# achilleasa/polaris

Hardware: AMD Instinct MI355X
Metric: Mrays/s (primary+indirect+occlusion rays traced / wall), Cornell box 512x512x128spp (higher is better)
Workload: dtype f32

## Files before the change

### polaris_amd/csrc/kernels.h

```cpp
#pragma once

#include <hip/hip_runtime.h>

#include <type_traits>

#include "builtin_probe.h"
#include "denoise.h"
#include "scene_layout.h"
#include "shading.h"
#include "temporal.h"
#include "variance.h"

namespace pol {

constexpr int WG = 256;
constexpr int kExitMarker = (int)0x80000000;

__device__ __forceinline__ float rcp_det(float x) {
	const float r = __builtin_amdgcn_rcpf(x);
	return __builtin_fmaf(__builtin_fmaf(-x, r, 1.0f), r, r);
}


__device__ __forceinline__ void rcp_dir(float dx, float dy, float dz, float &ix, float &iy, float &iz) {
// ... 1051 lines not shown
		uint32_t canon = 0;
		bool shade = tid < todo_rays;
		if (shade) canon = FIRST ? tid : canonical_index(pmask, (uint32_t)fbits(t4.w));
		if (!SORT && shade && A.prefilter) {
			const uint32_t fate = shade_fate(S, A, seed, [&]() { return pfx0 + canon; }, t4, h4.w);
			shade = fate == kFateLive;
			R.hit = fate == kFateRejected ? 1u : 0u;
		}
		if (shade) {
			shade_ray(S, A, s, seed, pfx0 + canon, d4, t4, h4, R, [&](float4 oo, float4 od, float4 oe) {
				const unsigned long long m = __ballot(true);
				const int first = __ffsll((long long)m) - 1;
				uint32_t at = 0;
				if ((int)lane == first) at = atomicAdd(&s_tot[1], (uint32_t)__popcll(m));
				const size_t d = base + (uint32_t)__builtin_amdgcn_readlane((int)at, first) + __popcll(m & below);
				st.occ_o[d] = oo; st.occ_d[d] = od; st.occ_e[d] = oe;
			});
		}
		const unsigned long long m_ind = __ballot(R.emit_ind);
		const unsigned long long mh = __ballot(R.hit != 0), mm = __ballot(R.miss != 0), me = __ballot(R.emit != 0);
		uint32_t at_ind = 0;
		if (lane == 0) {
			if (m_ind) at_ind = atomicAdd(&s_tot[0], (uint32_t)__popcll(m_ind));
			if (mh) atomicAdd(&s_tot[2], (uint32_t)__popcll(mh));
			if (mm) atomicAdd(&s_tot[3], (uint32_t)__popcll(mm));
			if (me) atomicAdd(&s_tot[4], (uint32_t)__popcll(me));
		}
		at_ind = __builtin_amdgcn_readfirstlane(at_ind);
		if (R.emit_ind) {
			atomicOr(&s_emit[canon >> 5], 1u << (canon & 31));
			const size_t d = base + at_ind + __popcll(m_ind & below);
			R.thr.w = ibits((int)canon);
			store_ray_o(st, d, R.ro); st.ray_d[d] = R.rd; st.thr[d] = R.thr;
		}
	}
	__threadfence_block();
	uint32_t arrived = 0;
	if (lane == 0) arrived = atomicAdd(&s_tot[5], 1u);
	if (__builtin_amdgcn_readfirstlane(arrived) == 3u) {
		__threadfence_block();
		if (lane == 0) {
			st.cnt_ray[blockIdx.x] = s_tot[0];
			st.cnt_occ[blockIdx.x] = s_tot[1];
			st.wg_stat[blockIdx.x] = s_tot[2] | (s_tot[3] << 10) | (s_tot[4] << 20);
		}
		if (lane < 8) A.emask_out[(size_t)blockIdx.x * 8 + lane] = s_emit[lane];
	}
}

constexpr int kSparseGroup = 8;
constexpr uint32_t kWaveQueue = 128;
static_assert(kWaveQueue >= 127 && (kWaveQueue & (kWaveQueue - 1)) == 0, "63 descriptors left by a shade pass + 64 of a screen pass; a ring indexed by masking");
static_assert(kSparseGroup <= 256 && WG <= 256, "a descriptor is chunk in group << 16 | slot << 8 | canonical index");
template <bool LDS>
__global__ __launch_bounds__(WG) __attribute__((amdgpu_waves_per_eu(4, 4)))
void k_shade_wave(Streams st, SceneDev Sg, ShadeArgs A, uint32_t num_chunks) {
	constexpr int G = kSparseGroup;
	__shared__ ShadeLds lds;
	__shared__ uint32_t wg_cursor;
	__shared__ uint32_t w_emit[4][G][8];
	__shared__ uint32_t w_cnt[4][G][3];
	__shared__ uint32_t w_queue[4][kWaveQueue];
	if (threadIdx.x == 0) wg_cursor = 0;
	for (uint32_t i = threadIdx.x; i < 4 * G * 8; i += WG) (&w_emit[0][0][0])[i] = 0;
	for (uint32_t i = threadIdx.x; i < 4 * G * 3; i += WG) (&w_cnt[0][0][0])[i] = 0;
	const SceneT<LDS> S = stage_scene<LDS>(Sg, lds);
	const uint32_t lane = threadIdx.x & 63, wave = threadIdx.x >> 6;
	const unsigned long long below = (1ull << lane) - 1ull;
	const uint32_t wgs_per_sample = A.Npad / WG;
	const uint32_t num_groups = (num_chunks + G - 1) / G;
	for (;;) {
		uint32_t c = 0;
		if (lane == 0) c = atomicAdd(&wg_cursor, 1u);
		const uint32_t group = blockIdx.x + __builtin_amdgcn_readfirstlane(c) * gridDim.x;
		if (group >= num_groups) break;
		const uint32_t chunk0 = group * G;
		const uint32_t my_cnt = (lane < (uint32_t)G && chunk0 + lane < num_chunks) ? st.cnt_ray[chunk0 + lane] : 0u;
		uint32_t incl = my_cnt;
#pragma unroll
		for (int d = 1; d < G; d <<= 1) {
			const uint32_t up = __shfl_up(incl, d);
			if ((int)lane >= d) incl += up;
		}
		const uint32_t excl = incl - my_cnt;
		const uint32_t total = (uint32_t)__builtin_amdgcn_readlane((int)incl, G - 1);
		uint32_t q_head = 0, q_tail = 0;
		auto shade_pass = [&]() {
			const uint32_t n = min(q_tail - q_head, 64u);
			const bool live = lane < n;
			__builtin_amdgcn_fence(__ATOMIC_RELEASE, "wavefront");
			__builtin_amdgcn_wave_barrier();
			__builtin_amdgcn_fence(__ATOMIC_ACQUIRE, "wavefront");
			const uint32_t desc = live ? w_queue[wave][(q_head + lane) & (kWaveQueue - 1)] : 0u;
			q_head += n;
			const uint32_t k = desc >> 16, idx = (desc >> 8) & 255u, canon = desc & 255u;
			const uint32_t chunk = chunk0 + k;
			const size_t base = (size_t)chunk * WG;
			ShadeOut R;
			R.emit_ind = false;
			R.hit = R.miss = R.emit = 0;
			if (live) {
				const uint32_t s = chunk / wgs_per_sample;
				const uint32_t seed = A.seeds[(size_t)(A.first_sample + s) * A.seed_stride + 1 + A.bounce];
				shade_ray(S, A, s, seed, st.pfx[chunk] + canon, st.ray_d[base + idx], st.thr[base + idx], load_hit(st, base + idx), R, [&](float4 oo, float4 od, float4 oe) {
					const size_t d = base + atomicAdd(&w_cnt[wave][k][1], 1u);
					st.occ_o[d] = oo; st.occ_d[d] = od; st.occ_e[d] = oe;
				});
			}
			if (R.emit_ind) {
				atomicOr(&w_emit[wave][k][canon >> 5], 1u << (canon & 31));
				const size_t d = base + atomicAdd(&w_cnt[wave][k][0], 1u);
				R.thr.w = ibits((int)canon);
				store_ray_o(st, d, R.ro); st.ray_d[d] = R.rd; st.thr[d] = R.thr;
			}
			if (live && (R.hit | R.miss | R.emit) != 0) atomicAdd(&w_cnt[wave][k][2], R.hit | (R.miss << 10) | (R.emit << 20));
		};
		for (uint32_t j = 0; j < total; j += 64) {
			const uint32_t r = j + lane;
			uint32_t k = 0, first = 0;
#pragma unroll
			for (int q = 1; q < G; q++) {
				const uint32_t e = (uint32_t)__builtin_amdgcn_readlane((int)excl, q);
				if (r >= e) { k = q; first = e; }
			}
			bool keep = false;
			uint32_t desc = 0;
			if (r < total) {
				const uint32_t chunk = chunk0 + k, idx = r - first;
				const size_t base = (size_t)chunk * WG;
				const float4 t4 = st.thr[base + idx];
				const uint4 m0 = reinterpret_cast<const uint4 *>(A.emask_in)[(size_t)chunk * 2], m1 = reinterpret_cast<const uint4 *>(A.emask_in)[(size_t)chunk * 2 + 1];
				const uint32_t pmask[8] = {m0.x, m0.y, m0.z, m0.w, m1.x, m1.y, m1.z, m1.w};
				const uint32_t canon = canonical_index(pmask, (uint32_t)fbits(t4.w));
				uint32_t fate = kFateLive;
				if (A.prefilter) {
					const uint32_t seed = A.seeds[(size_t)(A.first_sample + chunk / wgs_per_sample) * A.seed_stride + 1 + A.bounce];
					fate = shade_fate(S, A, seed, [&]() { return st.pfx[chunk] + canon; }, t4, load_hit_word(st, base + idx));
				}
				if (fate == kFateRejected) atomicAdd(&w_cnt[wave][k][2], 1u);
				keep = fate == kFateLive;
				desc = k << 16 | idx << 8 | canon;
			}
			const unsigned long long mk = __ballot(keep);
			if (keep) w_queue[wave][(q_tail + (uint32_t)__popcll(mk & below)) & (kWaveQueue - 1)] = desc;
			q_tail += (uint32_t)__popcll(mk);
			if (q_tail - q_head >= 64u) shade_pass();
		}
		if (q_tail != q_head) shade_pass();
		if (lane < (uint32_t)G && chunk0 + lane < num_chunks) {
			st.cnt_ray[chunk0 + lane] = w_cnt[wave][lane][0];
			st.cnt_occ[chunk0 + lane] = w_cnt[wave][lane][1];
			st.wg_stat[chunk0 + lane] = w_cnt[wave][lane][2];
			w_cnt[wave][lane][0] = 0; w_cnt[wave][lane][1] = 0; w_cnt[wave][lane][2] = 0;
		}
		for (uint32_t i = lane; i < (uint32_t)G * 8; i += 64) {
			if (chunk0 + i / 8 < num_chunks) A.emask_out[(size_t)chunk0 * 8 + i] = (&w_emit[wave][0][0])[i];
			(&w_emit[wave][0][0])[i] = 0;
		}
	}
}

enum ProbeKind { kProbeBxdf = 0, kProbeTexture = 1, kProbeEmissive = 2, kProbeMaterial = 3 };
constexpr uint32_t kProbeIn[4] = {13, 2, 11, 8}, kProbeOut[4] = {11, 7, 9, 18};

template <bool LDS>
__global__ __launch_bounds__(WG) void k_probe(SceneDev Sg, int kind, uint32_t index, uint32_t n, const float *in, float *out) {
	__shared__ ShadeLds lds;
	const SceneT<LDS> S = stage_scene<LDS>(Sg, lds);
	const uint32_t i = blockIdx.x * WG + threadIdx.x;
	if (i >= n) return;
	if (kind == kProbeBxdf) {
		const float *p = in + (size_t)i * 13;
		float *o = out + (size_t)i * 11;
		Surf sf;
		sf.p = splat(0.0f); sf.n = mk3(p[0], p[1], p[2]); sf.uv = {p[3], p[4]};
		const f3 wi = mk3(p[5], p[6], p[7]), wo = mk3(p[10], p[11], p[12]);
		MatT<LDS> m;
		m.nd = S.nodes + index;
		m.type = m.nd->type;
		m.int_ior = m.nd->int_ior; m.ext_ior = m.nd->ext_ior;
		material_params(sf, m, S);
		f3 dir = splat(0.0f);
		float pdf = 0.0f;
		const f3 v = bxdf_sample(sf, m, S, f2{p[8], p[9]}, wi, dir, pdf);
		float pdf2;
		f3 ev;
		bxdf_pdf_eval(sf, m, S, wi, wo, true, pdf2, ev);
		o[0] = v.x; o[1] = v.y; o[2] = v.z; o[3] = dir.x; o[4] = dir.y; o[5] = dir.z; o[6] = pdf;
		o[7] = pdf2; o[8] = ev.x; o[9] = ev.y; o[10] = ev.z;
	} else if (kind == kProbeTexture) {
		const float *p = in + (size_t)i * 2;
		float *o = out + (size_t)i * 7;
		const TexQuad q = tex_fetch(f2{p[0], p[1]}, (int)index, S);
		const f3 c = quad_sample3(q), b = quad_bump3(q);
		o[0] = c.x; o[1] = c.y; o[2] = c.z; o[3] = c.x; o[4] = b.x; o[5] = b.y; o[6] = b.z;
	} else if (kind == kProbeMaterial) {
		const float *p = in + (size_t)i * 8;
		float *o = out + (size_t)i * 18;
		Surf sf;
		sf.p = splat(0.0f); sf.n = mk3(p[0], p[1], p[2]); sf.uv = {p[3], p[4]};
		Rng rng = {(uint32_t)fbits(p[5]), (uint32_t)fbits(p[6])};
		uint32_t flags = (uint32_t)fbits(p[7]);
		f3 tint = splat(1.0f);
		const MatT<LDS> m = select_material(index, sf, flags, tint, rng, S);
		o[0] = ibits((int)m.type); o[1] = m.int_ior; o[2] = m.ext_ior;
		o[3] = sf.n.x; o[4] = sf.n.y; o[5] = sf.n.z; o[6] = tint.x; o[7] = tint.y; o[8] = tint.z;
		o[9] = ibits((int)flags); o[10] = ibits((int)rng.sx); o[11] = ibits((int)rng.sy);
		for (int k = 0; k < 3; k++) { o[12 + k] = m.nd->k[k]; o[15 + k] = m.nd->t[k]; }
// ... 486 lines not shown
```

### polaris_amd/csrc/polaris_hip.hip

```cpp
#include <hip/hip_runtime.h>

#include <algorithm>
#include <atomic>
#include <chrono>
#include <condition_variable>
#include <cmath>
#include <cstdarg>
#include <cstdio>
#include <cstdlib>
#include <cstring>
#include <map>
#include <memory>
#include <mutex>
#include <string>
#include <vector>

#include <unistd.h>

#include "camera_state.h"
#include "device_mem.h"
#include "frame_sync.h"
#include "kernel_table.h"
#include "merge_plan.h"
#include "polaris_hip.h"
// ... 233 lines not shown
	}
};

}

struct polaris_hip_tracer {
	int device = 0;
	char pci_bus_id[32] = {};
	hipStream_t stream = nullptr;
	std::mutex mu;
	std::string error;
	uint64_t error_seq = 0;

	FrameAccum fa;
	DevArray<uchar4> framebuffer;

	DeviceScene ds;
	int opt_node_mode = -1;
	int opt_tiny_one = 1;
	int opt_lds_tris = -1;

	CameraState camera;

	FrameSync fs;
	int opt_instance_update = 0, opt_vertex_update = 0;
	std::atomic<bool> opt_moments{false};

	struct Pipe {
		DevStream q;
		size_t slots = 0;
		Streams st{};
		float4 *nee[POLARIS_MAX_BOUNCES] = {};
		uint8_t *vis[POLARIS_MAX_BOUNCES] = {};
		uint32_t *cnt_occ_b[POLARIS_MAX_BOUNCES] = {};
		uint32_t nee_bounces = 0;
		DevPool bufs;
		DevEvent done;
		void release() {
			bufs.clear();
			st = Streams{};
			slots = 0;
			nee_bounces = 0;
			for (auto &x : nee) x = nullptr;
			for (auto &x : vis) x = nullptr;
			for (auto &x : cnt_occ_b) x = nullptr;
		}
	};
	static constexpr int kMaxPipes = pol::kMaxPipes;
	Pipe pipe[kMaxPipes];
	DevArray<uint32_t> d_seeds;
	DevArray<unsigned long long> d_stats;
	DevArray<float4> d_cam_o;
	int num_cus = 256;
	DevArray<uint32_t> d_retag;

	TraceOptions opt;
	bool packet_primary = true;
	int opt_time_kernels = 0;
	int opt_max_leaf_tris = -1;

	struct Pending { const char *name; DevEvent a, b; };
	std::vector<Pending> pending;
	std::vector<Pending> merge_pending;
	std::vector<DevEvent> event_pool;
	std::map<std::string, KernelTimer> timers;
	std::map<std::string, const char *> timer_symbol;
	int last_shade_timer[POLARIS_MAX_BOUNCES] = {};
	uint64_t last_shade_counts[3 * POLARIS_MAX_BOUNCES] = {};
	DevEvent ev_start, ev_stop, ev_fork;
};

struct polaris_hip_peer {
	polaris_hip_tracer *owner = nullptr;
	uint32_t depth = 0, W = 0, H = 0;
	IpcMapping mem[POLARIS_IPC_MAX_DEPTH];
	DevEvent ev[POLARIS_IPC_MAX_DEPTH];
	PolarisPeerInfo info{};
	void drop_events() { for (auto &e : ev) e.reset(); }
};


namespace {

int fail(polaris_hip_tracer *h, int code, const char *fmt, ...) {
	char buf[1024];
	va_list ap;
	va_start(ap, fmt);
	vsnprintf(buf, sizeof buf, fmt, ap);
	va_end(ap);
	if (h) { h->error = buf; h->error_seq = ++g_error_seq; }
	g_thread_error = buf;
	return code;
}

#define HIP_TRY(h, expr)                                                                              \
	do {                                                                                              \
		hipError_t e_ = (expr);                                                                       \
		if (e_ != hipSuccess) return fail(h, POLARIS_E_DEVICE, "%s failed: %s", #expr, hipGetErrorString(e_)); \
	} while (0)

template <typename T>
int dev_alloc(polaris_hip_tracer *h, DevPool &pool, T **out, size_t count) {
	DevArray<char> a;
	HIP_TRY(h, a.alloc(std::max<size_t>(count * sizeof(T), 16)));
	*out = (T *)a.get();
	pool.push_back(std::move(a));
// ... 194 lines not shown
	const bool tiny = h->ds.node_mode == kNodesLdsAll;
	for (int any = 0; any < 2; any++)
		h->ds.trace[any] = TraceLaunch{tiny ? &kTraceTiny[any][h->ds.tiny_one] : &kTrace[any][h->ds.max_stack <= 16 ? 0 : (h->ds.max_stack <= 24 ? 1 : 2)][h->ds.node_mode == kNodesLdsTop],
		                            tiny ? kTinyBlock : WG, 0, 6};
}

hipError_t launch_trace(polaris_hip_tracer *h, const char *timer, bool any_hit, hipStream_t q, Streams st, uint32_t grid, uint32_t chunks, float4 *acc, bool camera = false) {
	const TraceLaunch &T = h->ds.trace[any_hit];
	uint32_t o_mask = ~0u;
	if (camera && !any_hit) { st.ray_o = h->d_cam_o; o_mask = 0u; }
	return launch(h, timer, q, *T.v, grid, (uint32_t)T.block, T.lds_bytes, st, h->ds.bvh, chunks, acc, h->d_stats, o_mask);
}

int plan_tiny_lds(polaris_hip_tracer *h, size_t n_slots) {
	const uint32_t rows = (uint32_t)std::max(1, h->ds.max_stack - (h->ds.bvh.root_is_instance ? 1 : 0));
	constexpr uint32_t kRowBytes = kTinyBlock * (uint32_t)sizeof(int16_t), kTriBytes = 9 * sizeof(float) + sizeof(uint32_t);
	const uint32_t nodes = h->ds.bvh.num_pairs * (uint32_t)sizeof(PairNode);
	hipDeviceProp_t prop;
	size_t lds_per_cu = 160 * 1024;
	if (hipGetDeviceProperties(&prop, h->device) == hipSuccess && prop.maxSharedMemoryPerMultiProcessor > 0) lds_per_cu = prop.maxSharedMemoryPerMultiProcessor;
	const size_t half = lds_per_cu / 2;
	const size_t slack = 256;
	auto stack_off = [&](uint32_t tris) { return std::max<uint32_t>(kRowBytes, (nodes + tris * kTriBytes + 15u) & ~15u); };
	if (stack_off(0) + rows * kRowBytes + slack > half) return fail(h, POLARIS_E_DEVICE, "tiny-scene mode: stack and tree do not fit half a CU's LDS (%zu bytes)", half);
	uint32_t tris = (uint32_t)std::min<size_t>(n_slots, (half - slack - rows * kRowBytes - nodes - 16) / kTriBytes);
	if (tris < n_slots / 2) tris = 0;
	if (h->opt_lds_tris >= 0) tris = std::min<uint32_t>(tris, (uint32_t)h->opt_lds_tris);
	for (;;) {
		h->ds.bvh.tiny_stack_off = stack_off(tris);
		h->ds.bvh.lds_tris = tris;
		h->ds.trace[0].lds_bytes = h->ds.trace[1].lds_bytes = h->ds.bvh.tiny_stack_off + rows * kRowBytes;
		int worst = 8;
		for (const TraceLaunch &T : h->ds.trace) {
			HIP_TRY(h, hipFuncSetAttribute(T.v->address(), hipFuncAttributeMaxDynamicSharedMemorySize, (int)(half - slack)));
			int n = 0;
			if (hipOccupancyMaxActiveBlocksPerMultiprocessor(&n, T.v->address(), T.block, T.lds_bytes) != hipSuccess) { (void)hipGetLastError(); n = 2; }
			worst = std::min(worst, n);
		}
		if (worst >= 2 || tris == 0) break;
		tris = tris > 32 ? tris - 32 : 0;
	}
	if (getenv("POLARIS_DEBUG")) fprintf(stderr, "[polaris] tiny mode: %u stack rows at %u, %u pair records, %u of %zu triangle records in LDS (%u bytes per workgroup)\n", rows, h->ds.bvh.tiny_stack_off, h->ds.bvh.num_pairs, h->ds.bvh.lds_tris, n_slots, h->ds.trace[0].lds_bytes);
	return POLARIS_OK;
}

int trace_occupancy(polaris_hip_tracer *h, bool any_hit) {
	const TraceLaunch &T = h->ds.trace[any_hit];
	int n = 0;
	if (hipOccupancyMaxActiveBlocksPerMultiprocessor(&n, T.v->address(), T.block, T.lds_bytes) != hipSuccess || n < 1) n = h->ds.node_mode == kNodesLdsAll ? 1 : (h->ds.max_stack <= 24 ? 6 : 5);
	if (getenv("POLARIS_DEBUG")) fprintf(stderr, "[polaris] k_trace<%d> node mode %d: %d resident workgroups of %d threads per CU\n", (int)any_hit, h->ds.node_mode, n, T.block);
	return std::min(n, 8);
}

TraceScene plan_scene(const polaris_hip_tracer *h) {
	TraceScene s;
	s.tiny = h->ds.node_mode == kNodesLdsAll;
	for (int any = 0; any < 2; any++) s.resident_per_cu[any] = h->ds.trace[any].resident_per_cu;
	s.tables_fit_lds = h->ds.scene.num_nodes <= kLdsMatNodes && h->ds.scene.num_emissives <= kLdsLights && h->ds.scene.num_textures <= kLdsTextures;
	s.emit_classes = h->ds.scene.emit_classes;
	s.tri_bits = h->ds.scene.tri_bits;
	s.packet_primary = h->packet_primary;
	s.num_cus = h->num_cus;
	s.lens = h->camera.lens_on();
	s.shutter = h->camera.shutter_on();
	return s;
}

hipError_t launch_traversal(polaris_hip_tracer *h, const char *timer, Traversal how, RayKind kind, hipStream_t q, const Streams &st, uint32_t persistent_grid, uint32_t chunks, float4 *acc) {
	const bool any_hit = kind == RayKind::AnyHit;
	if (how == Traversal::Packet)
		return launch(h, timer, q, kPacket[any_hit ? kPacketAnyHit : (kind == RayKind::Camera ? kPacketCamera : kPacketClosest)], chunks, WG, 0, st, h->ds.bvh, acc, h->d_stats, make_float3(h->camera.open.eye[0], h->camera.open.eye[1], h->camera.open.eye[2]));
	if (how == Traversal::Persistent) return launch_trace(h, timer, any_hit, q, st, persistent_grid, chunks, acc, kind == RayKind::Camera);
	if (any_hit) return launch(h, timer, q, kOcclusion, chunks, WG, 0, st, h->ds.bvh, acc, h->d_stats);
	return launch(h, timer, q, kIntersect, chunks, WG, 0, st, h->ds.bvh);
}

hipError_t launch_generate(polaris_hip_tracer *h, const char *timer, hipStream_t q, const Streams &st, uint32_t stride, uint32_t first_sample, uint32_t wgs, uint32_t N,
                           uint32_t Npad, uint32_t block_y, int zero_lsum, int write_origin) {
	const CameraDev c = camera_args(h);
	const uint32_t *seeds = h->d_seeds;
	switch (const Generator g = h->camera.generator()) {
	case Generator::Pinhole: return launch(h, timer, q, kGenerate, wgs, WG, 0, st, c.cam, seeds, stride, first_sample, N, Npad, h->fa.W, block_y, zero_lsum, write_origin);
	case Generator::Lens: return launch(h, timer, q, kGenerateLens, wgs, WG, 0, st, c.cam, c.lens, seeds, stride, first_sample, N, Npad, h->fa.W, block_y, zero_lsum);
	default: return launch(h, timer, q, kGenerateShutter[g == Generator::ShutterLens], wgs, WG, 0, st, c.cam, c.cam1, c.lens, c.lens1, seeds, stride, first_sample, N, Npad, h->fa.W, block_y, zero_lsum);
	}
}

const char *const kShadeTimer[4] ={"shade_first", "shade_sort", "shade_plain", "shade_wave"};

hipError_t launch_batch(polaris_hip_tracer *h, int p, const PolarisBlockRequest *r, const TracePlan &plan, uint32_t s0, uint32_t K, uint32_t N, hipEvent_t resolve_after) {
	hipError_t first_err = hipSuccess;
	auto note = [&](hipError_t e) { if (first_err == hipSuccess && e != hipSuccess) first_err = e; };
	polaris_hip_tracer::Pipe &P = h->pipe[p];
	const bool exact = plan.exact;
	const uint32_t B = plan.bounces, stride = 1 + B, Npad = plan.Npad;
	const uint32_t wgs_per_sample = Npad / WG, wgs = K * wgs_per_sample;
	hipStream_t q = P.q;
	P.st.hit12 = plan.hit12 ? 1u : 0u;
	P.st.o12 = plan.o12 ? 1u : 0u;
	note(launch_generate(h, "generate", q, P.st, stride, s0, wgs, N, Npad, r->block_y, exact ? 0 : 1, plan.generate_writes_origins ? 1 : 0));
	ShadeArgs A{};
	A.seeds = h->d_seeds; A.seed_stride = stride; A.first_sample = s0;
	A.N = N; A.Npad = Npad; A.W = h->fa.W; A.blockY = r->block_y;
	A.min_rr = r->min_bounces_for_rr;
	A.exact = exact ? 1 : 0;
	A.prefilter = plan.prefilter ? 1 : 0;
	A.acc = exact ? h->fa.current() : P.st.lsum;
	const uint32_t persistent = plan.trace_grid(false, wgs), persistent_occl = plan.trace_grid(true, wgs);
	for (uint32_t b = 0; b < B; b++) {
		const BouncePlan &pl = plan.bounce[b];
		Streams S = P.st;
		if (!exact) { S.occ_e = P.nee[b]; S.vis = P.vis[b]; S.cnt_occ = P.cnt_occ_b[b]; }
		float4 *const occl_acc = exact ? A.acc : nullptr;
		const RayKind closest = b == 0 ? plan.primary : RayKind::Closest;
		note(launch_traversal(h, traversal_timer(pl.isect, closest), pl.isect, closest, q, S, persistent, wgs, nullptr));
// ... 238 lines not shown
	if (!out) return fail(nullptr, POLARIS_E_BAD_ARGUMENT, "device_identity: out is null");
	if (out->struct_size != sizeof(PolarisDeviceIdentity))
		return fail(nullptr, POLARIS_E_BAD_ARGUMENT, "device_identity: struct_size %u, this library's PolarisDeviceIdentity has %zu bytes", out->struct_size, sizeof(PolarisDeviceIdentity));
	const int n = polaris_hip_device_count();
	if (index < 0 || index >= n) return fail(nullptr, POLARIS_E_NO_DEVICE, "device %d out of range (%d devices)", index, n);
	hipDeviceProp_t p;
	HIP_TRY(nullptr, hipGetDeviceProperties(&p, index));
	memset(out, 0, sizeof *out);
	out->struct_size = sizeof *out;
	out->hip_index = index;
	if (hipDeviceGetPCIBusId(out->pci_bus_id, (int)sizeof out->pci_bus_id, index) != hipSuccess) { (void)hipGetLastError(); out->pci_bus_id[0] = 0; }
	hipUUID u;
	if (hipDeviceGetUuid(&u, index) == hipSuccess) memcpy(out->uuid, u.bytes, 16);
	else (void)hipGetLastError();
	out->compute_units = (uint32_t)p.multiProcessorCount;
	out->clock_mhz = (uint32_t)(p.clockRate / 1000);
	out->global_mem_bytes = (uint64_t)p.totalGlobalMem;
	snprintf(out->name, sizeof out->name, "%s", p.name);
	snprintf(out->gcn_arch, sizeof out->gcn_arch, "%s", p.gcnArchName);
	return POLARIS_OK;
}

int polaris_hip_can_access_peer(int device, int peer_device, int *can) {
	if (!can) return fail(nullptr, POLARIS_E_BAD_ARGUMENT, "can_access_peer: out is null");
	*can = 0;
	const int n = polaris_hip_device_count();
	if (device < 0 || device >= n || peer_device < 0 || peer_device >= n) return fail(nullptr, POLARIS_E_NO_DEVICE, "can_access_peer: device %d / %d out of range (%d devices)", device, peer_device, n);
	if (device == peer_device) return POLARIS_OK;
	HIP_TRY(nullptr, hipDeviceCanAccessPeer(can, device, peer_device));
	return POLARIS_OK;
}

int polaris_hip_create(int device_index, polaris_hip_tracer **out) {
	if (!out) return fail(nullptr, POLARIS_E_BAD_ARGUMENT, "out handle pointer is null");
	*out = nullptr;
	int n = polaris_hip_device_count();
	if (device_index < 0 || device_index >= n)
		return fail(nullptr, POLARIS_E_NO_DEVICE, "device %d out of range (%d HIP devices visible)", device_index, n);
	polaris_hip_tracer *h = new polaris_hip_tracer();
	h->device = device_index;
	if (hipDeviceGetPCIBusId(h->pci_bus_id, (int)sizeof h->pci_bus_id, device_index) != hipSuccess) { (void)hipGetLastError(); h->pci_bus_id[0] = 0; }
	hipError_t e = hipSetDevice(device_index);
	for (int p = 0; p < polaris_hip_tracer::kMaxPipes && e == hipSuccess; p++) e = h->pipe[p].q.create(hipStreamCreateWithFlags, hipStreamNonBlocking);
	h->stream = h->pipe[0].q;
	for (int p = 0; p < polaris_hip_tracer::kMaxPipes && e == hipSuccess; p++) e = h->pipe[p].done.create(hipEventCreateWithFlags, hipEventDisableTiming);
	if (e == hipSuccess) e = h->ev_fork.create(hipEventCreateWithFlags, hipEventDisableTiming);
	if (e == hipSuccess) e = h->fa.q.create(hipStreamCreateWithFlags, hipStreamNonBlocking);
	if (e == hipSuccess) e = h->fa.ev_merged.create(hipEventCreateWithFlags, hipEventDisableTiming);
	if (e == hipSuccess) e = h->d_stats.alloc(ST_COUNT);
	if (e == hipSuccess) e = h->d_cam_o.alloc(1);
	if (e == hipSuccess) {
		hipDeviceProp_t p;
		if (hipGetDeviceProperties(&p, device_index) == hipSuccess && p.multiProcessorCount > 0) h->num_cus = p.multiProcessorCount;
	}
	if (e == hipSuccess) e = h->ev_start.create(hipEventCreate);
	if (e == hipSuccess) e = h->ev_stop.create(hipEventCreate);
	if (e != hipSuccess) {
		fail(nullptr, POLARIS_E_DEVICE, "creating tracer on device %d: %s", device_index, hipGetErrorString(e));
		delete h;
		return POLARIS_E_DEVICE;
	}
	*out = h;
	return POLARIS_OK;
}

void polaris_hip_destroy(polaris_hip_tracer *h) {
	if (!h) return;
	{
		std::lock_guard<std::mutex> lk(h->mu);
		(void)hipSetDevice(h->device);
		if (h->stream) (void)hipStreamSynchronize(h->stream);
		for (int p = 1; p < polaris_hip_tracer::kMaxPipes; p++)
			if (h->pipe[p].q) (void)hipStreamSynchronize(h->pipe[p].q);
		if (h->fa.q) (void)hipStreamSynchronize(h->fa.q);
		collect_timers(h);
		std::lock_guard<std::mutex> lk_merge(h->fa.mu);
	}
	delete h;
}

const char *polaris_hip_last_error(polaris_hip_tracer *h) {
	if (!h) return g_thread_error.c_str();
	thread_local std::string copy;
	uint64_t seq;
	{
		std::lock_guard<std::mutex> lk(h->mu);
		copy = h->error;
		seq = h->error_seq;
	}
	{
		std::lock_guard<std::mutex> lk(h->fa.mu);
		if (h->fa.error_seq > seq) copy = h->fa.error;
	}
	return copy.c_str();
}

int polaris_hip_resize(polaris_hip_tracer *h, uint32_t frame_w, uint32_t frame_h) {
	if (!h) return fail(nullptr, POLARIS_E_BAD_ARGUMENT, "handle is null");
	std::lock_guard<std::mutex> lk(h->mu);
	if (frame_w == 0 || frame_h == 0 || (uint64_t)frame_w * frame_h > (1ull << 28))
		return fail(h, POLARIS_E_BAD_ARGUMENT, "bad frame dimensions %ux%u", frame_w, frame_h);
	HIP_TRY(h, hipSetDevice(h->device));
	std::lock_guard<std::mutex> lk_merge(h->fa.mu);
	HIP_TRY(h, sync_all(h));
	h->fa.release();
	h->fs.resized();
// ... 170 lines not shown
	if (!s.refusal.empty()) return fail(h, POLARIS_E_BAD_ARGUMENT, "%s", s.refusal.c_str());
	const bool drop = (s.todo & kCamDropHistory) && h->fs.tp.max_history;
	if (drop || eye) HIP_TRY(h, hipSetDevice(h->device));
	if (drop) HIP_TRY(h, hipStreamSynchronize(h->stream));
	if (eye) {
		const float4 o4 = make_float4(eye[0], eye[1], eye[2], kFltMax);
		HIP_TRY(h, hipMemcpy(h->d_cam_o, &o4, sizeof o4, hipMemcpyHostToDevice));
	}
	if (drop) h->fs.lens_changed();
	if (s.todo & kCamMoved) h->fs.camera_moved(h->camera.open);
	h->camera = s.next;
	return POLARIS_OK;
}

int polaris_hip_set_camera(polaris_hip_tracer *h, const float eye[3], const float fr[16]) {
	if (!h) return fail(nullptr, POLARIS_E_BAD_ARGUMENT, "handle is null");
	std::lock_guard<std::mutex> lk(h->mu);
	return apply_camera_step(h, h->camera.set_camera(eye, fr), eye);
}

int polaris_hip_set_lens(polaris_hip_tracer *h, const PolarisLensParams *p) {
	if (!h) return fail(nullptr, POLARIS_E_BAD_ARGUMENT, "handle is null");
	std::lock_guard<std::mutex> lk(h->mu);
	return apply_camera_step(h, h->camera.set_lens(p));
}

int polaris_hip_set_shutter(polaris_hip_tracer *h, const PolarisShutterParams *p) {
	if (!h) return fail(nullptr, POLARIS_E_BAD_ARGUMENT, "handle is null");
	std::lock_guard<std::mutex> lk(h->mu);
	return apply_camera_step(h, h->camera.set_shutter(p));
}

int polaris_hip_set_option(polaris_hip_tracer *h, const char *key, int64_t value) {
	if (!h) return fail(nullptr, POLARIS_E_BAD_ARGUMENT, "handle is null");
	std::lock_guard<std::mutex> lk(h->mu);
	if (!key) return fail(h, POLARIS_E_BAD_ARGUMENT, "option key is null");
	const std::string k(key);
	if (k == "samples_per_batch") h->opt.samples_per_batch = value < 0 ? 0 : value;
	else if (k == "exact_accumulate") {
		if (value != 0 && h->opt_moments) return fail(h, POLARIS_E_UNSUPPORTED, "exact_accumulate has no per-sample radiance: it cannot be combined with moments");
		h->opt.exact = value != 0;
	} else if (k == "moments") {
		if (value != 0 && h->opt.exact) return fail(h, POLARIS_E_UNSUPPORTED, "moments need per-sample radiance: exact_accumulate cannot keep them");
		if (value == 0 && h->fs.va.sigma_variance != 0.0f) return fail(h, POLARIS_E_BAD_ARGUMENT, "moments cannot be turned off while variance guidance is on");
		h->opt_moments = value != 0;
	}
	else if (k == "packet_primary") { h->opt.packet_primary = value < 0 ? -1 : (value != 0); if (value >= 0) h->packet_primary = value != 0; }
	else if (k == "packet_shadow") h->opt.packet_shadow = (int)std::max<int64_t>(0, std::min<int64_t>(value, POLARIS_MAX_BOUNCES));
	else if (k == "time_kernels") h->opt_time_kernels = value != 0;
	else if (k == "node_mode") h->opt_node_mode = (int)std::max<int64_t>(-1, std::min<int64_t>(value, 2));
	else if (k == "traversal") h->opt.traversal = value != 0;
	else if (k == "shade_wave") h->opt.shade_wave = value != 0;
	else if (k == "shade_wave_from") h->opt.shade_wave_from = (int)std::max<int64_t>(-1, std::min<int64_t>(value, POLARIS_MAX_BOUNCES));
	else if (k == "shade_wgs_per_cu") h->opt.shade_wgs_per_cu = (int)std::max<int64_t>(1, std::min<int64_t>(value, 64));
	else if (k == "stage_lds") h->opt.stage_lds = value != 0;
	else if (k == "shade_prefilter") h->opt.shade_prefilter = value != 0;
	else if (k == "shade_sort") h->opt.shade_sort = (int)std::max<int64_t>(-1, std::min<int64_t>(value, POLARIS_MAX_BOUNCES));
	else if (k == "ipc_staged") h->fa.ipc_staged = value != 0;
	else if (k == "overlap") h->opt.overlap = (int)std::max<int64_t>(1, std::min<int64_t>(value, polaris_hip_tracer::kMaxPipes));
	else if (k == "trace_grid") h->opt.trace_grid = (int)std::max<int64_t>(0, std::min<int64_t>(value, 1 << 20));
	else if (k == "trace_wgs_per_cu") h->opt.trace_wgs_per_cu = (int)std::max<int64_t>(0, std::min<int64_t>(value, 64));
	else if (k == "tiny_one") h->opt_tiny_one = value != 0;
	else if (k == "hit12") h->opt.hit12 = value != 0;
	else if (k == "o12") h->opt.o12 = value != 0;
	else if (k == "lds_tris") h->opt_lds_tris = (int)std::max<int64_t>(-1, std::min<int64_t>(value, 1 << 20));
	else if (k == "object_motion") {
		if (value != 0 && value != 1) return fail(h, POLARIS_E_BAD_ARGUMENT, "object_motion is 0 or 1");
		if ((int)value != h->fs.opt_object_motion) {
			HIP_TRY(h, hipSetDevice(h->device));
			HIP_TRY(h, hipStreamSynchronize(h->stream));
			h->fs.set_object_motion((int)value);
			if (value && h->ds.have_scene)
				if (int rc = read_back_instances(h)) return rc;
		}
	}
	else if (k == "vertex_motion") {
		if (value != 0 && value != 1) return fail(h, POLARIS_E_BAD_ARGUMENT, "vertex_motion is 0 or 1");
		if ((int)value != h->fs.opt_vertex_motion) {
			HIP_TRY(h, hipSetDevice(h->device));
			HIP_TRY(h, hipStreamSynchronize(h->stream));
			h->fs.set_vertex_motion((int)value);
		}
	}
	else if (k == "guide_specular") {
		if (value < 0 || value > 8) return fail(h, POLARIS_E_BAD_ARGUMENT, "guide_specular is 0..8");
		if ((int)value != h->fs.opt_guide_specular) h->fs.set_guide_specular((int)value);
	}
	else if (k == "instance_update") {
		if (value != 0 && value != 1) return fail(h, POLARIS_E_BAD_ARGUMENT, "instance_update is 0 or 1");
		h->opt_instance_update = (int)value;
	}
	else if (k == "vertex_update") {
		if (value != 0 && value != 1) return fail(h, POLARIS_E_BAD_ARGUMENT, "vertex_update is 0 or 1");
		h->opt_vertex_update = (int)value;
	}
	else if (k == "max_leaf_tris") h->opt_max_leaf_tris = (int)std::max<int64_t>(-1, std::min<int64_t>(value, 1 << 20));
	else return fail(h, POLARIS_E_BAD_ARGUMENT, "unknown option '%s'", key);
	return POLARIS_OK;
}

int polaris_hip_trace(polaris_hip_tracer *h, const PolarisBlockRequest *r, const uint32_t *seeds, size_t n_seeds,
                      PolarisTraceStats *stats) {
	if (!h) return fail(nullptr, POLARIS_E_BAD_ARGUMENT, "handle is null");
	std::lock_guard<std::mutex> lk(h->mu);
	struct ResetAnnounce {
		FrameAccum &fa; bool due;
		~ResetAnnounce() { if (due) (void)fa.reset_frame(false); }
// ... 1028 lines not shown
```

### polaris_amd/csrc/trace_plan.h

```cpp
#pragma once

#include <algorithm>
#include <cstddef>
#include <cstdint>

#include "polaris_types.h"

namespace pol {

constexpr uint32_t kPlanChunk = 256;
constexpr uint32_t kPlanSparseGroup = 8;
constexpr uint32_t kPlanTinyBlock = 1024;
constexpr int kMaxPipes = 8;

struct TraceOptions {
	int64_t samples_per_batch = 0;
	int exact = 0;
	int overlap = 4;
	int packet_shadow = 0;
	int packet_primary = -1;
	int traversal = 1;
	int trace_wgs_per_cu = 0;
	int trace_grid = 0;
	int stage_lds = 1;
	int shade_wave = 1;
	int shade_wgs_per_cu = 4;
	int shade_wave_from = -1;
	int shade_prefilter = 1;
	int shade_sort = -1;
	int hit12 = 1;
	int o12 = 1;
};

struct TraceScene {
	bool tiny = false;
	int resident_per_cu[2] = {6, 6};
	bool tables_fit_lds = false;
	uint32_t emit_classes = 0;
	uint32_t tri_bits = 0;
	bool packet_primary = true;
	int num_cus = 256;
	bool lens = false;
	bool shutter = false;
};

enum class RayKind { Camera, Closest, AnyHit };
enum class Traversal { Packet, Persistent, Plain };

inline Traversal traversal_unless_packet(bool packet, const TraceOptions &o) { return packet ? Traversal::Packet : (o.traversal ? Traversal::Persistent : Traversal::Plain); }
inline Traversal batch_traversal(const TraceOptions &o, const TraceScene &s, RayKind kind, uint32_t bounce) {
	return traversal_unless_packet(kind == RayKind::AnyHit ? (int)bounce < o.packet_shadow : (bounce == 0 && s.packet_primary), o);
}
inline Traversal probe_traversal(const TraceOptions &o, RayKind kind) {
	return traversal_unless_packet(kind == RayKind::AnyHit ? o.packet_shadow > 0 : o.packet_primary == 1, o);
}
inline Traversal tap_traversal(const TraceScene &s) { return s.packet_primary ? Traversal::Packet : Traversal::Plain; }
inline const char *traversal_timer(Traversal how, RayKind kind) {
	return kind == RayKind::AnyHit ? "occlusion" : (how == Traversal::Packet ? "intersect_packet" : "intersect");
}
inline uint32_t probe_grid(const TraceScene &s, bool any_hit, uint32_t wgs) {
	return std::min<uint32_t>(wgs, (uint32_t)s.num_cus * (uint32_t)std::max(1, s.resident_per_cu[any_hit]));
}
inline bool tables_staged(const TraceOptions &o, const TraceScene &s) { return o.stage_lds && s.tables_fit_lds; }

inline size_t slot_bytes(uint32_t nee_bounces) { return 144 + 17 * (size_t)std::max(1u, nee_bounces); }
constexpr uint32_t kBatchPathBudget = 32u << 20;
constexpr int64_t kMaxSamplesPerBatch = 4096;
constexpr uint32_t kWaveRouletteGroupsPerCu = 8;

enum ShadeKernel { kShadeFirst, kShadeSort, kShadePlain, kShadeByWave };

struct BouncePlan {
	Traversal isect = Traversal::Persistent, occl = Traversal::Persistent;
	ShadeKernel shade = kShadeFirst;
};

struct TracePlan {
	TraceOptions opt;
	TraceScene scene;
	uint32_t spp = 0, bounces = 0, min_rr = 0, Npad = kPlanChunk;

	bool exact = false;
	bool k_chosen = false;
	uint32_t K = 1;
	uint32_t n_batches = 0;
	int n_pipes = 1;
	bool staged = false;
	bool moments = false, prefilter = true, hit12 = true, o12 = true;
	bool generate_writes_origins = true;
	RayKind primary = RayKind::Camera;
	BouncePlan bounce[POLARIS_MAX_BOUNCES];

	uint32_t pipes_wanted() const { return (uint32_t)std::max(1, std::min(opt.overlap, kMaxPipes)); }
	bool overlapping() const { return pipes_wanted() > 1 && !exact; }

	void set_batch(uint32_t k) {
		K = k;
		n_batches = spp ? (spp + K - 1) / K : 0;
		n_pipes = exact ? 1 : (int)std::max<uint32_t>(1u, std::min<uint32_t>((uint32_t)opt.overlap, n_batches));
		plan_shading();
	}

	bool wants_memory_clamp() const { return !exact && !k_chosen && K > 1; }
	size_t bytes_needed(uint32_t k) const {
		return (size_t)k * Npad * slot_bytes(bounces) * std::min<size_t>(pipes_wanted(), (spp + k - 1) / k);
	}
	void clamp_to_memory(size_t available) {
		if (!wants_memory_clamp()) return;
		const size_t budget = available / 10 * 9;
		uint32_t k = K;
		while (k > 1 && bytes_needed(k) > budget) k = (k + 1) / 2;
		set_batch(k);
	}
	bool shrink() {
		if (exact || k_chosen || K == 1) return false;
		set_batch((K + 1) / 2);
		return true;
	}

	uint32_t trace_grid(bool any_hit, uint32_t wgs) const {
		uint32_t per_cu = (uint32_t)std::max(1, scene.resident_per_cu[any_hit]);
		if (overlapping() && per_cu > 2) per_cu = std::max(2u, per_cu * 2u / 3u);
		if (scene.tiny && overlapping() && per_cu == 2 && (uint64_t)wgs < 4ull * (uint64_t)scene.num_cus * per_cu * (kPlanTinyBlock / 64))
			per_cu = 1;
		if (opt.trace_wgs_per_cu > 0) per_cu = (uint32_t)opt.trace_wgs_per_cu;
		if (opt.trace_grid > 0) return std::min<uint32_t>(wgs, (uint32_t)opt.trace_grid);
		return std::min<uint32_t>(wgs, (uint32_t)scene.num_cus * per_cu);
	}
	uint32_t shade_wave_grid(uint32_t wgs) const {
		const uint32_t groups = (wgs + kPlanSparseGroup - 1) / kPlanSparseGroup;
		return std::max(1u, std::min<uint32_t>((groups + 3) / 4, (uint32_t)scene.num_cus * (uint32_t)std::max(1, opt.shade_wgs_per_cu)));
	}

private:
	void plan_shading() {
		int wave_from = opt.shade_wave_from;
		if (wave_from < 0) {
			wave_from = (int)min_rr + 1;
			const uint64_t batch_chunks = (uint64_t)K * (Npad / kPlanChunk);
			const uint64_t groups = (batch_chunks + kPlanSparseGroup - 1) / kPlanSparseGroup;
			if (opt.shade_prefilter && (scene.emit_classes & 0xFFFFu) != 0xFFFFu && groups >= (uint64_t)kWaveRouletteGroupsPerCu * (uint64_t)scene.num_cus)
				wave_from = (int)min_rr;
		}
		for (uint32_t b = 0; b < bounces; b++) {
			const bool wave = opt.shade_wave && b > 0 && (int)b >= wave_from;
			const bool sorted = b > 0 && scene.tri_bits < 31 && (int)b >= (opt.shade_sort >= 0 ? opt.shade_sort : 1);
			bounce[b].shade = wave ? kShadeByWave : (b == 0 ? kShadeFirst : (sorted ? kShadeSort : kShadePlain));
		}
	}
};

inline TracePlan plan_trace(const TraceOptions &opt, const TraceScene &scene, bool moments, uint32_t spp, uint32_t bounces, uint32_t min_rr, uint32_t Npad) {
	TracePlan p;
	p.opt = opt; p.scene = scene;
	p.spp = spp; p.bounces = bounces; p.min_rr = min_rr; p.Npad = Npad;
	p.exact = opt.exact != 0;
	p.k_chosen = opt.samples_per_batch > 0;
	p.staged = tables_staged(opt, scene);
	p.moments = moments; p.prefilter = opt.shade_prefilter != 0; p.hit12 = opt.hit12 != 0; p.o12 = opt.o12 != 0;
	const bool own_origins = scene.lens || scene.shutter;
	p.generate_writes_origins = own_origins || !(bounces > 0 && (scene.packet_primary || opt.traversal));
	p.primary = own_origins ? RayKind::Closest : RayKind::Camera;
	for (uint32_t b = 0; b < bounces; b++) {
		p.bounce[b].isect = batch_traversal(opt, scene, b == 0 ? p.primary : RayKind::Closest, b);
		p.bounce[b].occl = batch_traversal(opt, scene, RayKind::AnyHit, b);
	}
	uint32_t K = 1;
	if (!p.exact) {
		if (p.k_chosen) K = (uint32_t)std::min<int64_t>(opt.samples_per_batch, kMaxSamplesPerBatch);
		else K = std::min<uint32_t>(std::max<uint32_t>(1u, kBatchPathBudget / Npad), std::max(1u, (spp + 1) / 2));
		K = std::max<uint32_t>(1u, std::min(K, std::max(spp, 1u)));
	}
	p.set_batch(K);
	return p;
}

}
```

Before: 16840.

## Restructure wave-shading loop, cache per-chunk metadata in LDS, size grid by occupancy

Rewrites the k_shade_wave inner loop as a single state machine that alternates between screening rays and shading queued descriptors, instead of a nested lambda call. Per-chunk seed, sample index and prefix are read once into LDS. Offsets are rebased to the group's slot window, and the chunk scan uses DPP. The kernel's waves-per-EU target goes from 4 to 5, and the grid is now sized from the measured resident workgroups per CU so groups are spread over balanced rounds. The aim is lower register pressure and higher occupancy, at the risk of spills or weaker latency hiding per wave.

```diff
diff --git a/polaris_amd/csrc/kernels.h b/polaris_amd/csrc/kernels.h
--- a/polaris_amd/csrc/kernels.h
+++ b/polaris_amd/csrc/kernels.h
@@ -1127,8 +1127,33 @@
 constexpr uint32_t kWaveQueue = 128;
 static_assert(kWaveQueue >= 127 && (kWaveQueue & (kWaveQueue - 1)) == 0, "63 descriptors left by a shade pass + 64 of a screen pass; a ring indexed by masking");
 static_assert(kSparseGroup <= 256 && WG <= 256, "a descriptor is chunk in group << 16 | slot << 8 | canonical index");
+constexpr uint32_t kNoDesc = 0xFFFFFFFFu;
+__device__ __forceinline__ Streams streams_at(Streams st, size_t slot0) {
+	st.ray_o = reinterpret_cast<float4 *>(reinterpret_cast<char *>(st.ray_o) + slot0 * (st.o12 ? 12u : 16u));
+	st.hit = reinterpret_cast<float4 *>(reinterpret_cast<char *>(st.hit) + slot0 * (st.hit12 ? 12u : 16u));
+	st.ray_d += slot0; st.thr += slot0;
+	st.occ_o += slot0; st.occ_d += slot0; st.occ_e += slot0;
+	st.pfx += slot0 / WG;
+	return st;
+}
+__device__ __forceinline__ uint32_t desc_again(uint32_t desc) {
+	asm volatile("" : "+v"(desc));
+	return desc;
+}
+__device__ __forceinline__ uint32_t lane_again() {
+	uint32_t l;
+	asm volatile("v_mbcnt_lo_u32_b32 %0, -1, 0\n\tv_mbcnt_hi_u32_b32 %0, -1, %0" : "=v"(l));
+	return l;
+}
+__device__ __forceinline__ uint32_t uniform_again(uint32_t u) {
+	asm volatile("" : "+s"(u));
+	return u;
+}
+#ifndef POLARIS_SHADE_WAVE_WAVES
+#define POLARIS_SHADE_WAVE_WAVES 5
+#endif
 template <bool LDS>
-__global__ __launch_bounds__(WG) __attribute__((amdgpu_waves_per_eu(4, 4)))
+__global__ __launch_bounds__(WG) __attribute__((amdgpu_waves_per_eu(POLARIS_SHADE_WAVE_WAVES, POLARIS_SHADE_WAVE_WAVES)))
 void k_shade_wave(Streams st, SceneDev Sg, ShadeArgs A, uint32_t num_chunks) {
 	constexpr int G = kSparseGroup;
 	__shared__ ShadeLds lds;
@@ -1136,99 +1161,122 @@
 	__shared__ uint32_t w_emit[4][G][8];
 	__shared__ uint32_t w_cnt[4][G][3];
 	__shared__ uint32_t w_queue[4][kWaveQueue];
+	__shared__ uint32_t w_pre[4][G];
+	__shared__ uint32_t w_meta[4][G][4];
 	if (threadIdx.x == 0) wg_cursor = 0;
 	for (uint32_t i = threadIdx.x; i < 4 * G * 8; i += WG) (&w_emit[0][0][0])[i] = 0;
 	for (uint32_t i = threadIdx.x; i < 4 * G * 3; i += WG) (&w_cnt[0][0][0])[i] = 0;
 	const SceneT<LDS> S = stage_scene<LDS>(Sg, lds);
-	const uint32_t lane = threadIdx.x & 63, wave = threadIdx.x >> 6;
-	const unsigned long long below = (1ull << lane) - 1ull;
-	const uint32_t wgs_per_sample = A.Npad / WG;
+	const uint32_t wave = (uint32_t)__builtin_amdgcn_readfirstlane((int)(threadIdx.x >> 6));
 	const uint32_t num_groups = (num_chunks + G - 1) / G;
 	for (;;) {
+		const uint32_t lane = lane_again();
 		uint32_t c = 0;
 		if (lane == 0) c = atomicAdd(&wg_cursor, 1u);
 		const uint32_t group = blockIdx.x + __builtin_amdgcn_readfirstlane(c) * gridDim.x;
 		if (group >= num_groups) break;
 		const uint32_t chunk0 = group * G;
-		const uint32_t my_cnt = (lane < (uint32_t)G && chunk0 + lane < num_chunks) ? st.cnt_ray[chunk0 + lane] : 0u;
-		uint32_t incl = my_cnt;
-#pragma unroll
-		for (int d = 1; d < G; d <<= 1) {
-			const uint32_t up = __shfl_up(incl, d);
-			if ((int)lane >= d) incl += up;
-		}
-		const uint32_t excl = incl - my_cnt;
-		const uint32_t total = (uint32_t)__builtin_amdgcn_readlane((int)incl, G - 1);
-		uint32_t q_head = 0, q_tail = 0;
-		auto shade_pass = [&]() {
-			const uint32_t n = min(q_tail - q_head, 64u);
-			const bool live = lane < n;
+		const Streams sg = streams_at(st, (size_t)chunk0 * WG);
+		uint32_t total;
+		{
+			const bool has = lane < (uint32_t)G && chunk0 + lane < num_chunks;
+			uint32_t my_cnt = 0, s = 0, seed = 0, pfx0 = 0;
+			if (has) {
+				s = (chunk0 + lane) / uniform_again(A.Npad / WG);
+				my_cnt = st.cnt_ray[chunk0 + lane];
+				seed = A.seeds[(size_t)(A.first_sample + s) * A.seed_stride + 1 + A.bounce];
+				pfx0 = sg.pfx[lane];
+			}
+			uint32_t incl = my_cnt;
+			incl += (uint32_t)__builtin_amdgcn_update_dpp(0, (int)incl, 0x111, 0xf, 0xf, false);
+			incl += (uint32_t)__builtin_amdgcn_update_dpp(0, (int)incl, 0x112, 0xf, 0xf, false);
+			incl += (uint32_t)__builtin_amdgcn_update_dpp(0, (int)incl, 0x114, 0xf, 0xf, false);
+			static_assert(G == 8, "three steps scan lanes 0 .. 7 of a row of 16");
+			if (lane < (uint32_t)G) {
+				w_pre[wave][lane] = incl - my_cnt;
+				w_meta[wave][lane][0] = s; w_meta[wave][lane][1] = seed; w_meta[wave][lane][2] = pfx0;
+			}
+			total = (uint32_t)__builtin_amdgcn_readlane((int)incl, G - 1);
 			__builtin_amdgcn_fence(__ATOMIC_RELEASE, "wavefront");
 			__builtin_amdgcn_wave_barrier();
 			__builtin_amdgcn_fence(__ATOMIC_ACQUIRE, "wavefront");
-			const uint32_t desc = live ? w_queue[wave][(q_head + lane) & (kWaveQueue - 1)] : 0u;
-			q_head += n;
-			const uint32_t k = desc >> 16, idx = (desc >> 8) & 255u, canon = desc & 255u;
-			const uint32_t chunk = chunk0 + k;
-			const size_t base = (size_t)chunk * WG;
-			ShadeOut R;
-			R.emit_ind = false;
-			R.hit = R.miss = R.emit = 0;
-			if (live) {
-				const uint32_t s = chunk / wgs_per_sample;
-				const uint32_t seed = A.seeds[(size_t)(A.first_sample + s) * A.seed_stride + 1 + A.bounce];
-				shade_ray(S, A, s, seed, st.pfx[chunk] + canon, st.ray_d[base + idx], st.thr[base + idx], load_hit(st, base + idx), R, [&](float4 oo, float4 od, float4 oe) {
-					const size_t d = base + atomicAdd(&w_cnt[wave][k][1], 1u);
-					st.occ_o[d] = oo; st.occ_d[d] = od; st.occ_e[d] = oe;
-				});
-			}
-			if (R.emit_ind) {
-				atomicOr(&w_emit[wave][k][canon >> 5], 1u << (canon & 31));
-				const size_t d = base + atomicAdd(&w_cnt[wave][k][0], 1u);
-				R.thr.w = ibits((int)canon);
-				store_ray_o(st, d, R.ro); st.ray_d[d] = R.rd; st.thr[d] = R.thr;
-			}
-			if (live && (R.hit | R.miss | R.emit) != 0) atomicAdd(&w_cnt[wave][k][2], R.hit | (R.miss << 10) | (R.emit << 20));
-		};
-		for (uint32_t j = 0; j < total; j += 64) {
-			const uint32_t r = j + lane;
-			uint32_t k = 0, first = 0;
+		}
+		uint32_t q_head = 0, q_tail = 0;
+		uint32_t j = 0;
+		for (;;) {
+			const uint32_t queued = q_tail - q_head;
+			if (j < total && queued < 64u) {
+				const uint32_t r = j + lane_again();
+				j += 64;
+				uint32_t k = 0, first = 0;
 #pragma unroll
-			for (int q = 1; q < G; q++) {
-				const uint32_t e = (uint32_t)__builtin_amdgcn_readlane((int)excl, q);
-				if (r >= e) { k = q; first = e; }
-			}
-			bool keep = false;
-			uint32_t desc = 0;
-			if (r < total) {
-				const uint32_t chunk = chunk0 + k, idx = r - first;
-				const size_t base = (size_t)chunk * WG;
-				const float4 t4 = st.thr[base + idx];
-				const uint4 m0 = reinterpret_cast<const uint4 *>(A.emask_in)[(size_t)chunk * 2], m1 = reinterpret_cast<const uint4 *>(A.emask_in)[(size_t)chunk * 2 + 1];
-				const uint32_t pmask[8] = {m0.x, m0.y, m0.z, m0.w, m1.x, m1.y, m1.z, m1.w};
-				const uint32_t canon = canonical_index(pmask, (uint32_t)fbits(t4.w));
-				uint32_t fate = kFateLive;
-				if (A.prefilter) {
-					const uint32_t seed = A.seeds[(size_t)(A.first_sample + chunk / wgs_per_sample) * A.seed_stride + 1 + A.bounce];
-					fate = shade_fate(S, A, seed, [&]() { return st.pfx[chunk] + canon; }, t4, load_hit_word(st, base + idx));
+				for (int q = 1; q < G; q++) {
+					const uint32_t e = w_pre[wave][q];
+					if (r >= e) { k = q; first = e; }
 				}
-				if (fate == kFateRejected) atomicAdd(&w_cnt[wave][k][2], 1u);
-				keep = fate == kFateLive;
-				desc = k << 16 | idx << 8 | canon;
-			}
-			const unsigned long long mk = __ballot(keep);
-			if (keep) w_queue[wave][(q_tail + (uint32_t)__popcll(mk & below)) & (kWaveQueue - 1)] = desc;
-			q_tail += (uint32_t)__popcll(mk);
-			if (q_tail - q_head >= 64u) shade_pass();
-		}
-		if (q_tail != q_head) shade_pass();
-		if (lane < (uint32_t)G && chunk0 + lane < num_chunks) {
-			st.cnt_ray[chunk0 + lane] = w_cnt[wave][lane][0];
-			st.cnt_occ[chunk0 + lane] = w_cnt[wave][lane][1];
-			st.wg_stat[chunk0 + lane] = w_cnt[wave][lane][2];
-			w_cnt[wave][lane][0] = 0; w_cnt[wave][lane][1] = 0; w_cnt[wave][lane][2] = 0;
-		}
-		for (uint32_t i = lane; i < (uint32_t)G * 8; i += 64) {
+				bool keep = false;
+				uint32_t desc = 0;
+				if (r < total) {
+					const uint32_t idx = r - first;
+					const uint32_t at = k * WG + idx;
+					const float4 t4 = sg.thr[at];
+					const uint4 *em = reinterpret_cast<const uint4 *>(A.emask_in) + (size_t)chunk0 * 2;
+					const uint4 m0 = em[k * 2], m1 = em[k * 2 + 1];
+					const uint32_t pmask[8] = {m0.x, m0.y, m0.z, m0.w, m1.x, m1.y, m1.z, m1.w};
+					const uint32_t canon = canonical_index(pmask, (uint32_t)fbits(t4.w));
+					uint32_t fate = kFateLive;
+					if (A.prefilter) {
+						fate = shade_fate(S, A, w_meta[wave][k][1], [&]() { return w_meta[wave][k][2] + canon; }, t4, load_hit_word(sg, at));
+					}
+					if (fate == kFateRejected) atomicAdd(&w_cnt[wave][k][2], 1u);
+					keep = fate == kFateLive;
+					desc = at << 8 | canon;
+				}
+				const unsigned long long mk = __ballot(keep);
+				const uint32_t rank = __builtin_amdgcn_mbcnt_hi((uint32_t)(mk >> 32), __builtin_amdgcn_mbcnt_lo((uint32_t)mk, 0u));
+				if (keep) w_queue[wave][(q_tail + rank) & (kWaveQueue - 1)] = desc;
+				q_tail += (uint32_t)__popcll(mk);
+			} else if (queued != 0u) {
+				const uint32_t n = min(queued, 64u);
+				__builtin_amdgcn_fence(__ATOMIC_RELEASE, "wavefront");
+				__builtin_amdgcn_wave_barrier();
+				__builtin_amdgcn_fence(__ATOMIC_ACQUIRE, "wavefront");
+				const uint32_t ql = lane_again();
+				const uint32_t desc = ql < n ? w_queue[wave][(q_head + ql) & (kWaveQueue - 1)] : kNoDesc;
+				q_head += n;
+				ShadeOut R;
+				R.emit_ind = false;
+				R.hit = R.miss = R.emit = 0;
+				if (desc != kNoDesc) {
+					SceneT<LDS> Sp = S;
+					Sp.num_emissives = uniform_again(S.num_emissives);
+					const uint32_t k = desc >> 16, at = desc >> 8, canon = desc & 255u;
+					shade_ray(Sp, A, w_meta[wave][k][0], w_meta[wave][k][1], w_meta[wave][k][2] + canon, sg.ray_d[at], sg.thr[at], load_hit(sg, at), R, [&](float4 oo, float4 od, float4 oe) {
+						const uint32_t k2 = desc_again(desc) >> 16;
+						const uint32_t d = (k2 * WG + atomicAdd(&w_cnt[wave][k2][1], 1u)) & (G * WG - 1);
+						sg.occ_o[d] = oo; sg.occ_d[d] = od; sg.occ_e[d] = oe;
+					});
+				}
+				const uint32_t k = desc_again(desc) >> 16, canon = desc_again(desc) & 255u;
+				if (R.emit_ind) {
+					atomicOr(&w_emit[wave][k][canon >> 5], 1u << (canon & 31));
+					const uint32_t d = (k * WG + atomicAdd(&w_cnt[wave][k][0], 1u)) & (G * WG - 1);
+					R.thr.w = ibits((int)canon);
+					store_ray_o(sg, d, R.ro); sg.ray_d[d] = R.rd; sg.thr[d] = R.thr;
+				}
+				if ((R.hit | R.miss | R.emit) != 0) atomicAdd(&w_cnt[wave][k][2], R.hit | (R.miss << 10) | (R.emit << 20));
+			} else {
+				break;
+			}
+		}
+		const uint32_t pl = lane_again();
+		if (pl < (uint32_t)G && chunk0 + pl < num_chunks) {
+			st.cnt_ray[chunk0 + pl] = w_cnt[wave][pl][0];
+			st.cnt_occ[chunk0 + pl] = w_cnt[wave][pl][1];
+			st.wg_stat[chunk0 + pl] = w_cnt[wave][pl][2];
+			w_cnt[wave][pl][0] = 0; w_cnt[wave][pl][1] = 0; w_cnt[wave][pl][2] = 0;
+		}
+		for (uint32_t i = pl; i < (uint32_t)G * 8; i += 64) {
 			if (chunk0 + i / 8 < num_chunks) A.emask_out[(size_t)chunk0 * 8 + i] = (&w_emit[wave][0][0])[i];
 			(&w_emit[wave][0][0])[i] = 0;
 		}
diff --git a/polaris_amd/csrc/polaris_hip.hip b/polaris_amd/csrc/polaris_hip.hip
--- a/polaris_amd/csrc/polaris_hip.hip
+++ b/polaris_amd/csrc/polaris_hip.hip
@@ -309,6 +309,7 @@
 	DevArray<unsigned long long> d_stats;
 	DevArray<float4> d_cam_o;
 	int num_cus = 256;
+	int shade_wave_resident[2] = {5, 5};
 	DevArray<uint32_t> d_retag;
 
 	TraceOptions opt;
@@ -609,6 +610,13 @@
 	return std::min(n, 8);
 }
 
+int shade_wave_occupancy(bool lds) {
+	int n = 0;
+	if (hipOccupancyMaxActiveBlocksPerMultiprocessor(&n, kShadeWave[lds].address(), WG, 0) != hipSuccess || n < 1) { (void)hipGetLastError(); n = POLARIS_SHADE_WAVE_WAVES; }
+	if (getenv("POLARIS_DEBUG")) fprintf(stderr, "[polaris] k_shade_wave<%d>: %d resident workgroups of %d threads per CU\n", (int)lds, n, (int)WG);
+	return std::min(n, 8);
+}
+
 TraceScene plan_scene(const polaris_hip_tracer *h) {
 	TraceScene s;
 	s.tiny = h->ds.node_mode == kNodesLdsAll;
@@ -618,6 +626,7 @@
 	s.tri_bits = h->ds.scene.tri_bits;
 	s.packet_primary = h->packet_primary;
 	s.num_cus = h->num_cus;
+	for (int lds = 0; lds < 2; lds++) s.shade_wave_resident[lds] = h->shade_wave_resident[lds];
 	s.lens = h->camera.lens_on();
 	s.shutter = h->camera.shutter_on();
 	return s;
@@ -962,6 +971,7 @@
 	if (e == hipSuccess) {
 		hipDeviceProp_t p;
 		if (hipGetDeviceProperties(&p, device_index) == hipSuccess && p.multiProcessorCount > 0) h->num_cus = p.multiProcessorCount;
+		for (int lds = 0; lds < 2; lds++) h->shade_wave_resident[lds] = shade_wave_occupancy(lds != 0);
 	}
 	if (e == hipSuccess) e = h->ev_start.create(hipEventCreate);
 	if (e == hipSuccess) e = h->ev_stop.create(hipEventCreate);
@@ -1238,7 +1248,7 @@
 	else if (k == "traversal") h->opt.traversal = value != 0;
 	else if (k == "shade_wave") h->opt.shade_wave = value != 0;
 	else if (k == "shade_wave_from") h->opt.shade_wave_from = (int)std::max<int64_t>(-1, std::min<int64_t>(value, POLARIS_MAX_BOUNCES));
-	else if (k == "shade_wgs_per_cu") h->opt.shade_wgs_per_cu = (int)std::max<int64_t>(1, std::min<int64_t>(value, 64));
+	else if (k == "shade_wgs_per_cu") h->opt.shade_wgs_per_cu = (int)std::max<int64_t>(0, std::min<int64_t>(value, 64));
 	else if (k == "stage_lds") h->opt.stage_lds = value != 0;
 	else if (k == "shade_prefilter") h->opt.shade_prefilter = value != 0;
 	else if (k == "shade_sort") h->opt.shade_sort = (int)std::max<int64_t>(-1, std::min<int64_t>(value, POLARIS_MAX_BOUNCES));
diff --git a/polaris_amd/csrc/trace_plan.h b/polaris_amd/csrc/trace_plan.h
--- a/polaris_amd/csrc/trace_plan.h
+++ b/polaris_amd/csrc/trace_plan.h
@@ -24,7 +24,7 @@
 	int trace_grid = 0;
 	int stage_lds = 1;
 	int shade_wave = 1;
-	int shade_wgs_per_cu = 4;
+	int shade_wgs_per_cu = 0;
 	int shade_wave_from = -1;
 	int shade_prefilter = 1;
 	int shade_sort = -1;
@@ -40,6 +40,7 @@
 	uint32_t tri_bits = 0;
 	bool packet_primary = true;
 	int num_cus = 256;
+	int shade_wave_resident[2] = {5, 5};
 	bool lens = false;
 	bool shutter = false;
 };
@@ -129,7 +130,10 @@
 	}
 	uint32_t shade_wave_grid(uint32_t wgs) const {
 		const uint32_t groups = (wgs + kPlanSparseGroup - 1) / kPlanSparseGroup;
-		return std::max(1u, std::min<uint32_t>((groups + 3) / 4, (uint32_t)scene.num_cus * (uint32_t)std::max(1, opt.shade_wgs_per_cu)));
+		if (opt.shade_wgs_per_cu > 0) return std::max(1u, std::min<uint32_t>((groups + 3) / 4, (uint32_t)scene.num_cus * (uint32_t)opt.shade_wgs_per_cu));
+		const uint32_t waves = 4u * (uint32_t)scene.num_cus * (uint32_t)std::max(1, scene.shade_wave_resident[staged]);
+		const uint32_t rounds = std::max(1u, (groups + waves - 1) / waves);
+		return std::max(1u, (groups + 4u * rounds - 1) / (4u * rounds));
 	}
 
 private:
```

New measurement: 17040 (median of 6 runs). +1.2%, better.
